# giolucasd/ssrl-vit-mae-jepa

Hardware: AMD Instinct MI355X
Metric: images/sec pretrain step (fwd+bwd+opt), ViT-S/8 96px MAE, 1/2/4/8 MI355X (higher is better)
Workload: dtype bf16; 1 GPU; ViT-S/8 96px MAE (enc 384x12x6h, dec 192x2x6h, mask_ratio 0.75), batch 2000/GPU, full step; global_batch=2000, per_gpu_batch=2000, parallelism=dp1

## Files before the change

### __graft_entry__.py

```python
from __future__ import annotations

import os
import subprocess
import sys
from pathlib import Path

ROOT = Path(__file__).resolve().parent
if str(ROOT) not in sys.path:
    sys.path.insert(0, str(ROOT))


def build() -> None:
    env = dict(os.environ)
    env.setdefault("HIPCC", "/opt/rocm/bin/hipcc")
    jobs = str(min(8, os.cpu_count() or 1))
    subprocess.run(["make", "-C", str(ROOT / "ssrl_vit_mae_jepa_amd" / "csrc"), "-j", jobs, "ARCH=gfx950"], check=True, env=env)
    subprocess.run(["bash", str(ROOT / "tools" / "build_dbg_lib.sh"), "vmcnt0"], check=True, env=dict(env, JOBS=jobs))
    import oracle.mae_oracle
    import ssrl_vit_mae_jepa_amd
    print("build ok:", ssrl_vit_mae_jepa_amd.LIB_PATH)


def smoke() -> None:
    import torch
    from oracle import mae_oracle as O
    from ssrl_vit_mae_jepa_amd import MaskedAutoencoder

    torch.set_float32_matmul_precision("highest")
    dev = torch.device("cuda:0")
    cfg = O.YAML_TINY
    B = 4
    params = O.init_params(cfg, 73)
    O.randomize_params(params)
    images = O.synthetic_images(B, cfg)
    noise = O.make_noise(B, cfg.sequence_length, torch.Generator().manual_seed(74))
    loss_ref, grads_ref, aux = O.loss_and_grads(params, cfg, images, noise)
    for precision, tol in (("fp32", 1e-4), ("bf16", 2e-2)):
        model = MaskedAutoencoder(
            dict(image_size=cfg.image_size, patch_size=cfg.patch_size, in_chans=cfg.in_chans, engine_precision=precision),
            dict(embed_dim=cfg.embed_dim, depth=cfg.depth, num_heads=cfg.num_heads),
            dict(decoder_embed_dim=cfg.decoder_embed_dim, decoder_depth=cfg.decoder_depth, decoder_num_heads=cfg.decoder_num_heads))
        model.load_state_dict(params)
        model = model.to(dev)
        loss, keep, mask = model.loss_and_grads(images.to(dev), noise.to(dev), return_indices=True)
        torch.cuda.synchronize()
        assert torch.equal(keep.cpu(), aux["idx_keep"]) and torch.equal(mask.cpu(), aux["idx_mask"]), "mask indices differ"
        rel = abs(loss.item() - loss_ref.item()) / abs(loss_ref.item())
        assert rel <= tol, f"{precision}: loss {loss.item()} vs oracle {loss_ref.item()} (rel {rel:.2e})"
        g = model.named_flat_views(model.flat_grads)
        gn = sum(float(v.double().pow(2).sum()) for v in g.values()) ** 0.5
        gr = sum(float(v.double().pow(2).sum()) for v in grads_ref.values()) ** 0.5
        assert abs(gn - gr) <= max(50 * tol, 1e-3) * gr, f"{precision}: grad norm {gn} vs {gr}"
        print(f"smoke {precision}: loss {loss.item():.6f} (oracle {loss_ref.item():.6f}, rel {rel:.1e}), |g| {gn:.5f} vs {gr:.5f}")


if __name__ == "__main__":
    build()
    if len(sys.argv) > 1 and sys.argv[1] == "smoke":
        smoke()
```

### ssrl_vit_mae_jepa_amd/csrc/k_attention_mfma.hip

```cpp
#include "gemm_mfma.h"

#ifndef MAE_ATT_DMA_POLICY
#define MAE_ATT_DMA_POLICY 0
#endif
#ifdef MAE_ATT_NT
#define AT_ST store4_nt
#else
#define AT_ST store4
#endif

namespace mae {

namespace {

constexpr float kLog2e = 1.4426950408889634f;

template <int HD>
struct AT {
  static constexpr int RS = HD * 2 + 32;
  static constexpr int NKS = HD / 32;
  static constexpr int NDT = HD / 16;
  static constexpr int CPR = HD / 8;
};

template <int HD>
__device__ __forceinline__ void stage_image(char* s, const bf16* g, int64_t gs, int T, int Tp) {
  for (int c = threadIdx.x; c < Tp * AT<HD>::CPR; c += blockDim.x) {
    const int row = c / AT<HD>::CPR, cc = c - row * AT<HD>::CPR;
    uint4 v = uint4{0, 0, 0, 0};
    if (row < T) v = *reinterpret_cast<const uint4*>(g + row * gs + cc * 8);
    *reinterpret_cast<uint4*>(s + row * AT<HD>::RS + cc * 16) = v;
  }
}

template <int HD>
__device__ __forceinline__ void stage_image_dma(char* s, int img_bytes, const bf16* g, int64_t gs, int T, int wave, int nwaves, int lane, int cprv) {
  constexpr int SPR = AT<HD>::RS / 16;
  for (int blk = wave; blk * 1024 < img_bytes; blk += nwaves) {
    const int slot = blk * 64 + lane;
    int row = slot / SPR, c = slot - row * SPR;
    row = row < T ? row : T - 1;
    c = c < cprv ? c : cprv - 1;
    __builtin_amdgcn_global_load_lds((const __attribute__((address_space(1))) void*)(g + row * gs + c * 8),
                                     (__attribute__((address_space(3))) void*)(s + blk * 1024), 16, 0, MAE_ATT_DMA_POLICY);
  }
}

template <int HD>
__device__ __forceinline__ void zero_pad_chunks(char* s, int rows, int cprv) {
  const int npad = AT<HD>::CPR - cprv;
  for (int i = threadIdx.x; i < rows * npad; i += blockDim.x) {
    const int row = i / npad, c = cprv + (i - row * npad);
    *reinterpret_cast<uint4*>(s + row * AT<HD>::RS + c * 16) = uint4{0, 0, 0, 0};
  }
}

template <int HD, bool CL>
__device__ __forceinline__ bf16x8 rowfrag(const char* s, int row0, int ks, int lane, int rmax) {
  const int row = CL ? min(row0 + (lane & 15), rmax) : row0 + (lane & 15);
  return *reinterpret_cast<const bf16x8*>(s + row * AT<HD>::RS + (ks * 32 + 8 * (lane >> 4)) * 2);
}

template <int HD, bool CL>
__device__ __forceinline__ bf16x8 trfrag(const char* s, int j0, int c0, int lane, int rmax) {
  const int g = lane >> 4, q = (lane & 15) >> 2, p = lane & 3;
  const int r = j0 + 4 * g + q;
  const char* a = s + (CL ? min(r, rmax) : r) * AT<HD>::RS + (c0 + 4 * p) * 2;
  const char* a2 = CL ? s + min(r + 16, rmax) * AT<HD>::RS + (c0 + 4 * p) * 2 : a + 16 * AT<HD>::RS;
  const bf16x4 lo = __builtin_amdgcn_ds_read_tr16_b64_v4bf16((__attribute__((address_space(3))) bf16x4*)(a));
  const bf16x4 hi = __builtin_amdgcn_ds_read_tr16_b64_v4bf16((__attribute__((address_space(3))) bf16x4*)(a2));
  return bf16x8{lo[0], lo[1], lo[2], lo[3], hi[0], hi[1], hi[2], hi[3]};
}

__device__ __forceinline__ bf16x8 pack8(const f32x4& a, const f32x4& b) {
  return bf16x8{(bf16)a[0], (bf16)a[1], (bf16)a[2], (bf16)a[3], (bf16)b[0], (bf16)b[1], (bf16)b[2], (bf16)b[3]};
}

__device__ __forceinline__ float group_max(float v) {
  auto a = __builtin_amdgcn_permlane16_swap(__float_as_uint(v), __float_as_uint(v), false, false);
  v = fmaxf(__uint_as_float(a[0]), __uint_as_float(a[1]));
  auto b = __builtin_amdgcn_permlane32_swap(__float_as_uint(v), __float_as_uint(v), false, false);
  return fmaxf(__uint_as_float(b[0]), __uint_as_float(b[1]));
}
__device__ __forceinline__ float group_sum(float v) {
  auto a = __builtin_amdgcn_permlane16_swap(__float_as_uint(v), __float_as_uint(v), false, false);
  v = __uint_as_float(a[0]) + __uint_as_float(a[1]);
  auto b = __builtin_amdgcn_permlane32_swap(__float_as_uint(v), __float_as_uint(v), false, false);
  return __uint_as_float(b[0]) + __uint_as_float(b[1]);
}

}

__device__ __forceinline__ void first_generation_stagger(int stagger, int gen1) {
  if (stagger > 0 && (int)blockIdx.x >= 256 && (int)blockIdx.x < gen1) {
    const uint64_t t0 = wall_clock64(), wait = (uint64_t)(blockIdx.x >> 8) * stagger;
    while (wall_clock64() - t0 < wait) __builtin_amdgcn_s_sleep(4);
  }
}

__device__ __forceinline__ int att_block(int remap) {
  if (!remap) return (int)blockIdx.x;
  const int nb = (int)gridDim.x, bid = (int)blockIdx.x;
  const int q = nb >> 3, r = nb & 7, xcd = bid & 7, loc = bid >> 3;
  return (xcd < r ? xcd * (q + 1) : r * (q + 1) + (xcd - r) * q) + loc;
}

template <int HD> struct FwdCap { static constexpr int v = 512; };
template <int NCH> struct BwdCap { static constexpr int v = NCH == 0 ? 1024 : 512; };

template <int HD>
__device__ __forceinline__ bf16x8 rowfrag_global(const bf16* g, int64_t gs, int row0, int ks, int lane, int T) {
  int row = row0 + (lane & 15);
  row = row < T ? row : T - 1;
  return *reinterpret_cast<const bf16x8*>(g + row * gs + ks * 32 + 8 * (lane >> 4));
}

template <int HD, int NCH, bool FQ = false>
__global__ void __launch_bounds__(FwdCap<HD>::v) attn_fwd_mfma_kernel(const bf16* __restrict__ qkv, int T, int Tp, int H, float scale,
                                                            bf16* __restrict__ out, float* __restrict__ lse, int stagger, int gen1, int hdv, int remap) {
  extern __shared__ __attribute__((aligned(16))) char smem[];
  first_generation_stagger(stagger, gen1);
  constexpr bool CL = NCH >= 1 && NCH <= 3;
  const int Ti = CL ? (T + 15) & ~15 : Tp, rmax = Ti - 1;
  const int img = (Ti * AT<HD>::RS + 1023) & ~1023;
  char* sQ = smem;
  char* sK = FQ ? smem : sQ + img;
  char* sV = sK + img;
  const int vb = att_block(remap);
  const int b = vb / H, h = vb - b * H;
  const int64_t gs = 3ll * H * hdv;
  const int cprv = hdv >> 3;
  const bf16* base = qkv + (int64_t)b * T * gs + h * hdv;
  const int lane = threadIdx.x & 63, nwaves = blockDim.x >> 6;
  const int wave = __builtin_amdgcn_readfirstlane(threadIdx.x >> 6);
  if (!FQ) stage_image_dma<HD>(sQ, img, base, gs, T, wave, nwaves, lane, cprv);
  stage_image_dma<HD>(sK, img, base + (int64_t)H * hdv, gs, T, wave, nwaves, lane, cprv);
  stage_image_dma<HD>(sV, img, base + 2ll * H * hdv, gs, T, wave, nwaves, lane, cprv);
  asm volatile("s_waitcnt vmcnt(0)" ::: "memory");
  if (hdv < HD) {
    if (!FQ) zero_pad_chunks<HD>(sQ, Ti, cprv);
    zero_pad_chunks<HD>(sK, Ti, cprv);
    zero_pad_chunks<HD>(sV, Ti, cprv);
  }
  __syncthreads();
  const int g = lane >> 4, i = lane & 15;
  const float sl2 = scale * kLog2e;
  const int nq = (T + 15) >> 4, nchunks = NCH > 0 ? NCH : (Tp >> 5);
  for (int qt = wave; qt < nq; qt += nwaves) {
    bf16x8 qf[AT<HD>::NKS];
#pragma unroll
    for (int ks = 0; ks < AT<HD>::NKS; ++ks) qf[ks] = FQ ? rowfrag_global<HD>(base, gs, qt * 16, ks, lane, T) : rowfrag<HD, CL>(sQ, qt * 16, ks, lane, rmax);
    f32x4 oacc[AT<HD>::NDT];
#pragma unroll
    for (int dt = 0; dt < AT<HD>::NDT; ++dt) oacc[dt] = f32x4{0.f, 0.f, 0.f, 0.f};
    float m = -INFINITY, lsum = 0.f;
    if constexpr (NCH > 0) {
      constexpr int NC = NCH > 0 ? NCH : 1;
      f32x4 s0[NC], s1[NC];
#pragma unroll
      for (int c = 0; c < NC; ++c) {
        s0[c] = f32x4{0.f, 0.f, 0.f, 0.f}; s1[c] = s0[c];
#pragma unroll
        for (int ks = 0; ks < AT<HD>::NKS; ++ks) {
          s0[c] = __builtin_amdgcn_mfma_f32_16x16x32_bf16(rowfrag<HD, CL>(sK, c * 32, ks, lane, rmax), qf[ks], s0[c], 0, 0, 0);
          s1[c] = __builtin_amdgcn_mfma_f32_16x16x32_bf16(rowfrag<HD, CL>(sK, c * 32 + 16, ks, lane, rmax), qf[ks], s1[c], 0, 0, 0);
        }
      }
      {
        const int j0 = (NC - 1) * 32 + 4 * g;
#pragma unroll
        for (int r = 0; r < 4; ++r) {
          if (j0 + r >= T) s0[NC - 1][r] = -INFINITY;
          if (j0 + 16 + r >= T) s1[NC - 1][r] = -INFINITY;
        }
      }
      float mc = -INFINITY;
#pragma unroll
      for (int c = 0; c < NC; ++c)
        mc = fmaxf(mc, fmaxf(fmaxf(fmaxf(s0[c][0], s0[c][1]), fmaxf(s0[c][2], s0[c][3])), fmaxf(fmaxf(s1[c][0], s1[c][1]), fmaxf(s1[c][2], s1[c][3]))));
      m = group_max(mc);
      const float mn2 = m * sl2;
#pragma unroll
      for (int c = 0; c < NC; ++c) {
#pragma unroll
        for (int r = 0; r < 4; ++r) {
          s0[c][r] = __builtin_amdgcn_exp2f(fmaf(s0[c][r], sl2, -mn2));
          s1[c][r] = __builtin_amdgcn_exp2f(fmaf(s1[c][r], sl2, -mn2));
          lsum += s0[c][r] + s1[c][r];
        }
        const bf16x8 pf = pack8(s0[c], s1[c]);
#pragma unroll
        for (int dt = 0; dt < AT<HD>::NDT; ++dt)
          oacc[dt] = __builtin_amdgcn_mfma_f32_16x16x32_bf16(trfrag<HD, CL>(sV, c * 32, dt * 16, lane, rmax), pf, oacc[dt], 0, 0, 0);
      }
    } else {
    for (int c = 0; c < nchunks; ++c) {
      f32x4 s0 = {0.f, 0.f, 0.f, 0.f}, s1 = {0.f, 0.f, 0.f, 0.f};
#pragma unroll
      for (int ks = 0; ks < AT<HD>::NKS; ++ks) {
        s0 = __builtin_amdgcn_mfma_f32_16x16x32_bf16(rowfrag<HD, CL>(sK, c * 32, ks, lane, rmax), qf[ks], s0, 0, 0, 0);
        s1 = __builtin_amdgcn_mfma_f32_16x16x32_bf16(rowfrag<HD, CL>(sK, c * 32 + 16, ks, lane, rmax), qf[ks], s1, 0, 0, 0);
      }
      const int j0 = c * 32 + 4 * g;
      if (c * 32 + 32 > T) {
#pragma unroll
        for (int r = 0; r < 4; ++r) {
          if (j0 + r >= T) s0[r] = -INFINITY;
          if (j0 + 16 + r >= T) s1[r] = -INFINITY;
        }
      }
      float mc = fmaxf(fmaxf(fmaxf(s0[0], s0[1]), fmaxf(s0[2], s0[3])), fmaxf(fmaxf(s1[0], s1[1]), fmaxf(s1[2], s1[3])));
      mc = group_max(mc);
      const float mn = fmaxf(m, mc);
      const float mn2 = mn * sl2;
      const float alpha = __builtin_amdgcn_exp2f(m * sl2 - mn2);
      float ps = 0.f;
#pragma unroll
      for (int r = 0; r < 4; ++r) {
        s0[r] = __builtin_amdgcn_exp2f(fmaf(s0[r], sl2, -mn2));
        s1[r] = __builtin_amdgcn_exp2f(fmaf(s1[r], sl2, -mn2));
        ps += s0[r] + s1[r];
      }
      lsum = lsum * alpha + ps;
      const bf16x8 pf = pack8(s0, s1);
#pragma unroll
      for (int dt = 0; dt < AT<HD>::NDT; ++dt) {
        oacc[dt] *= alpha;
        oacc[dt] = __builtin_amdgcn_mfma_f32_16x16x32_bf16(trfrag<HD, CL>(sV, c * 32, dt * 16, lane, rmax), pf, oacc[dt], 0, 0, 0);
      }
      m = mn;
    }
    }
    lsum = group_sum(lsum);
    const float inv = 1.0f / lsum;
    const int tq = qt * 16 + i;
    if (tq < T) {
      bf16* po = out + ((int64_t)b * T + tq) * H * hdv + h * hdv + 4 * g;
#pragma unroll
      for (int dt = 0; dt < AT<HD>::NDT; ++dt)
        if (dt * 16 + 4 * g < hdv) AT_ST(po + dt * 16, oacc[dt] * inv);
      if (g == 0) lse[((int64_t)b * H + h) * T + tq] = m * scale + __logf(lsum);
    }
  }
}

template <int HD, int NCH, int PH = 0>
__global__ void __launch_bounds__(BwdCap<NCH>::v) attn_bwd_mfma_kernel(const bf16* __restrict__ qkv, const bf16* __restrict__ out,
                                                            const bf16* __restrict__ d_out, const float* __restrict__ lse, int T,
                                                            int Tp, int H, float scale, bf16* __restrict__ d_qkv, int stagger, int gen1, int hdv, int remap) {
  extern __shared__ __attribute__((aligned(16))) char smem[];
  first_generation_stagger(stagger, gen1);
  constexpr bool CL = NCH >= 1 && NCH <= 3;
  const int Ti = CL ? (T + 15) & ~15 : Tp, rmax = Ti - 1;
  const int img = (Ti * AT<HD>::RS + 1023) & ~1023;
  char* sQ = smem;
  char* sK = PH == 1 ? smem : sQ + img;
  char* sV = sK + img;
  char* sdO = PH == 2 ? smem + img : sV + img;
  float* sLse = reinterpret_cast<float*>(smem + (PH == 0 ? 4 : 2) * img);
  float* sD = sLse + Tp;
  const int vb = att_block(remap);
  const int b = vb / H, h = vb - b * H;
  const int64_t gs = 3ll * H * hdv, os = (int64_t)H * hdv;
  const int cprv = hdv >> 3;
  const bf16* base = qkv + (int64_t)b * T * gs + h * hdv;
  const bf16* obase = out + (int64_t)b * T * os + h * hdv;
  const bf16* dobase = d_out + (int64_t)b * T * os + h * hdv;
  bf16* dbase = d_qkv + (int64_t)b * T * gs + h * hdv;
  const int lane = threadIdx.x & 63, nwaves = blockDim.x >> 6;
  const int wave = __builtin_amdgcn_readfirstlane(threadIdx.x >> 6);
  if (PH != 1) stage_image_dma<HD>(sQ, img, base, gs, T, wave, nwaves, lane, cprv);
  if (PH != 2) stage_image_dma<HD>(sK, img, base + os, gs, T, wave, nwaves, lane, cprv);
  if (PH != 2) stage_image_dma<HD>(sV, img, base + 2 * os, gs, T, wave, nwaves, lane, cprv);
  if (PH != 1) stage_image_dma<HD>(sdO, img, dobase, os, T, wave, nwaves, lane, cprv);
  constexpr bool DPM = NCH > 0 && PH == 0;
  constexpr int CPR = AT<HD>::CPR, PF = 4;
  const int total = Tp * CPR;
  const bool pf = !DPM && PH == 0 && total <= PF * (int)blockDim.x;
  if (DPM) {
    for (int t = threadIdx.x; t < Tp; t += blockDim.x) {
      sLse[t] = t < T ? lse[((int64_t)b * H + h) * T + t] * kLog2e : 1e30f;
      sD[t] = 0.f;
    }
  }
  bf16x8 o_pf[PF];
  float l_pf[PF];
  if (pf) {
#pragma unroll
    for (int it = 0; it < PF; ++it) {
      const int idx = it * blockDim.x + threadIdx.x;
      const int t = idx / CPR, cc = idx - t * CPR;
      const bool live = idx < total && t < T && cc < cprv;
      const int tc = live ? t : 0;
      o_pf[it] = *reinterpret_cast<const bf16x8*>(obase + tc * os + (live ? cc : 0) * 8);
      l_pf[it] = lse[((int64_t)b * H + h) * T + tc];
    }
  }
  asm volatile("s_waitcnt vmcnt(0)" ::: "memory");
  if (hdv < HD) {
    if (PH != 1) zero_pad_chunks<HD>(sQ, Ti, cprv);
    if (PH != 2) zero_pad_chunks<HD>(sK, Ti, cprv);
    if (PH != 2) zero_pad_chunks<HD>(sV, Ti, cprv);
    if (PH != 1) zero_pad_chunks<HD>(sdO, Ti, cprv);
  }
  __syncthreads();
  if (pf) {
#pragma unroll
    for (int it = 0; it < PF; ++it) {
      const int idx = it * blockDim.x + threadIdx.x;
      const int t = idx / CPR, cc = idx - t * CPR;
      float D = 0.f;
      if (idx < total && t < T && cc < cprv) {
        const bf16x8 a = *reinterpret_cast<const bf16x8*>(sdO + t * AT<HD>::RS + cc * 16);
#pragma unroll
        for (int e = 0; e < 8; ++e) D = fmaf((float)a[e], (float)o_pf[it][e], D);
      }
#pragma unroll
      for (int off = CPR / 2; off > 0; off >>= 1) D += __shfl_xor(D, off, 64);
      if (idx < total && cc == 0) {
        sD[t] = D;
        sLse[t] = t < T ? l_pf[it] * kLog2e : 1e30f;
      }
    }
  } else if (!DPM) {
    for (int base = 0; base < total; base += blockDim.x) {
      const int idx = base + threadIdx.x;
      const int t = idx / CPR, cc = idx - t * CPR;
      float D = 0.f;
      if (idx < total && t < T && cc < cprv) {
        const bf16x8 a = PH == 1 ? *reinterpret_cast<const bf16x8*>(dobase + t * os + cc * 8) : *reinterpret_cast<const bf16x8*>(sdO + t * AT<HD>::RS + cc * 16);
        const bf16x8 o = *reinterpret_cast<const bf16x8*>(obase + t * os + cc * 8);
#pragma unroll
        for (int e = 0; e < 8; ++e) D = fmaf((float)a[e], (float)o[e], D);
      }
#pragma unroll
      for (int off = CPR / 2; off > 0; off >>= 1) D += __shfl_xor(D, off, 64);
      if (idx < total && cc == 0) {
        sD[t] = D;
        sLse[t] = t < T ? lse[((int64_t)b * H + h) * T + t] * kLog2e : 1e30f;
      }
    }
  }
  if (!DPM) __syncthreads();
  const int g = lane >> 4, i = lane & 15;
  const float sl2 = scale * kLog2e;
  const int nt16 = (T + 15) >> 4, nchunks = NCH > 0 ? NCH : (Tp >> 5);

#ifdef MAE_DBG_ATT_NO_A
  if (T < 0)
#endif
  if (PH != 2)
  for (int qt = wave; qt < nt16; qt += nwaves) {
    bf16x8 qf[AT<HD>::NKS], dof[AT<HD>::NKS];
#pragma unroll
    for (int ks = 0; ks < AT<HD>::NKS; ++ks) {
      qf[ks] = PH == 1 ? rowfrag_global<HD>(base, gs, qt * 16, ks, lane, T) : rowfrag<HD, CL>(sQ, qt * 16, ks, lane, rmax);
      dof[ks] = PH == 1 ? rowfrag_global<HD>(dobase, os, qt * 16, ks, lane, T) : rowfrag<HD, CL>(sdO, qt * 16, ks, lane, rmax);
    }
    const float li = sLse[qt * 16 + i];
    f32x4 dq[AT<HD>::NDT];
#pragma unroll
    for (int dt = 0; dt < AT<HD>::NDT; ++dt) dq[dt] = f32x4{0.f, 0.f, 0.f, 0.f};
    if constexpr (DPM) {
      constexpr int NC = NCH > 0 ? NCH : 1;
      f32x4 P0[NC], P1[NC], G0[NC], G1[NC];
      float dpart = 0.f;
#pragma unroll
      for (int c = 0; c < NC; ++c) {
        f32x4 s0 = {0.f, 0.f, 0.f, 0.f}, s1 = s0;
        G0[c] = s0; G1[c] = s0;
#pragma unroll
        for (int ks = 0; ks < AT<HD>::NKS; ++ks) {
          s0 = __builtin_amdgcn_mfma_f32_16x16x32_bf16(rowfrag<HD, CL>(sK, c * 32, ks, lane, rmax), qf[ks], s0, 0, 0, 0);
          s1 = __builtin_amdgcn_mfma_f32_16x16x32_bf16(rowfrag<HD, CL>(sK, c * 32 + 16, ks, lane, rmax), qf[ks], s1, 0, 0, 0);
          G0[c] = __builtin_amdgcn_mfma_f32_16x16x32_bf16(rowfrag<HD, CL>(sV, c * 32, ks, lane, rmax), dof[ks], G0[c], 0, 0, 0);
          G1[c] = __builtin_amdgcn_mfma_f32_16x16x32_bf16(rowfrag<HD, CL>(sV, c * 32 + 16, ks, lane, rmax), dof[ks], G1[c], 0, 0, 0);
        }
        if (c == NC - 1) {
          const int j0 = c * 32 + 4 * g;
#pragma unroll
          for (int r = 0; r < 4; ++r) {
            if (j0 + r >= T) s0[r] = -INFINITY;
            if (j0 + 16 + r >= T) s1[r] = -INFINITY;
          }
        }
#pragma unroll
        for (int r = 0; r < 4; ++r) {
          P0[c][r] = __builtin_amdgcn_exp2f(fmaf(s0[r], sl2, -li));
          P1[c][r] = __builtin_amdgcn_exp2f(fmaf(s1[r], sl2, -li));
          dpart = fmaf(P0[c][r], G0[c][r], dpart);
          dpart = fmaf(P1[c][r], G1[c][r], dpart);
        }
      }
      const float Di = group_sum(dpart);
      if (g == 0) sD[qt * 16 + i] = Di;
#pragma unroll
      for (int c = 0; c < NC; ++c) {
        f32x4 d0, d1;
#pragma unroll
        for (int r = 0; r < 4; ++r) {
          d0[r] = P0[c][r] * (G0[c][r] - Di);
          d1[r] = P1[c][r] * (G1[c][r] - Di);
        }
        const bf16x8 dsf = pack8(d0, d1);
#pragma unroll
        for (int dt = 0; dt < AT<HD>::NDT; ++dt)
          dq[dt] = __builtin_amdgcn_mfma_f32_16x16x32_bf16(trfrag<HD, CL>(sK, c * 32, dt * 16, lane, rmax), dsf, dq[dt], 0, 0, 0);
      }
    } else {
    const float Di = sD[qt * 16 + i];
#pragma unroll
    for (int c = 0; c < nchunks; ++c) {
      f32x4 s0 = {0.f, 0.f, 0.f, 0.f}, s1 = s0, p0 = s0, p1 = s0;
#pragma unroll
      for (int ks = 0; ks < AT<HD>::NKS; ++ks) {
        s0 = __builtin_amdgcn_mfma_f32_16x16x32_bf16(rowfrag<HD, CL>(sK, c * 32, ks, lane, rmax), qf[ks], s0, 0, 0, 0);
        s1 = __builtin_amdgcn_mfma_f32_16x16x32_bf16(rowfrag<HD, CL>(sK, c * 32 + 16, ks, lane, rmax), qf[ks], s1, 0, 0, 0);
        p0 = __builtin_amdgcn_mfma_f32_16x16x32_bf16(rowfrag<HD, CL>(sV, c * 32, ks, lane, rmax), dof[ks], p0, 0, 0, 0);
        p1 = __builtin_amdgcn_mfma_f32_16x16x32_bf16(rowfrag<HD, CL>(sV, c * 32 + 16, ks, lane, rmax), dof[ks], p1, 0, 0, 0);
      }
      const int j0 = c * 32 + 4 * g;
      if (NCH > 0 ? c == NCH - 1 : c * 32 + 32 > T) {
#pragma unroll
        for (int r = 0; r < 4; ++r) {
          if (j0 + r >= T) s0[r] = -INFINITY;
          if (j0 + 16 + r >= T) s1[r] = -INFINITY;
        }
      }
#pragma unroll
      for (int r = 0; r < 4; ++r) {
        const float pa = __builtin_amdgcn_exp2f(fmaf(s0[r], sl2, -li));
        const float pb = __builtin_amdgcn_exp2f(fmaf(s1[r], sl2, -li));
        s0[r] = pa * (p0[r] - Di);
        s1[r] = pb * (p1[r] - Di);
      }
      const bf16x8 dsf = pack8(s0, s1);
#pragma unroll
      for (int dt = 0; dt < AT<HD>::NDT; ++dt)
        dq[dt] = __builtin_amdgcn_mfma_f32_16x16x32_bf16(trfrag<HD, CL>(sK, c * 32, dt * 16, lane, rmax), dsf, dq[dt], 0, 0, 0);
    }
    }
    const int tq = qt * 16 + i;
    if (tq < T) {
#pragma unroll
      for (int dt = 0; dt < AT<HD>::NDT; ++dt)
        if (dt * 16 + 4 * g < hdv) AT_ST(dbase + tq * gs + dt * 16 + 4 * g, dq[dt] * scale);
    }
  }
  if (DPM) __syncthreads();

#ifdef MAE_DBG_ATT_NO_B
  if (T < 0)
#endif
  if (PH != 1)
  for (int jt = wave; jt < nt16; jt += nwaves) {
    bf16x8 kf[AT<HD>::NKS], vf[AT<HD>::NKS];
#pragma unroll
    for (int ks = 0; ks < AT<HD>::NKS; ++ks) {
      kf[ks] = PH == 2 ? rowfrag_global<HD>(base + os, gs, jt * 16, ks, lane, T) : rowfrag<HD, CL>(sK, jt * 16, ks, lane, rmax);
      vf[ks] = PH == 2 ? rowfrag_global<HD>(base + 2 * os, gs, jt * 16, ks, lane, T) : rowfrag<HD, CL>(sV, jt * 16, ks, lane, rmax);
    }
    f32x4 dk[AT<HD>::NDT], dv[AT<HD>::NDT];
#pragma unroll
    for (int dt = 0; dt < AT<HD>::NDT; ++dt) { dk[dt] = f32x4{0.f, 0.f, 0.f, 0.f}; dv[dt] = dk[dt]; }
#pragma unroll
    for (int c = 0; c < nchunks; ++c) {
      f32x4 s0 = {0.f, 0.f, 0.f, 0.f}, s1 = s0, p0 = s0, p1 = s0;
#pragma unroll
      for (int ks = 0; ks < AT<HD>::NKS; ++ks) {
        s0 = __builtin_amdgcn_mfma_f32_16x16x32_bf16(rowfrag<HD, CL>(sQ, c * 32, ks, lane, rmax), kf[ks], s0, 0, 0, 0);
        s1 = __builtin_amdgcn_mfma_f32_16x16x32_bf16(rowfrag<HD, CL>(sQ, c * 32 + 16, ks, lane, rmax), kf[ks], s1, 0, 0, 0);
        p0 = __builtin_amdgcn_mfma_f32_16x16x32_bf16(rowfrag<HD, CL>(sdO, c * 32, ks, lane, rmax), vf[ks], p0, 0, 0, 0);
        p1 = __builtin_amdgcn_mfma_f32_16x16x32_bf16(rowfrag<HD, CL>(sdO, c * 32 + 16, ks, lane, rmax), vf[ks], p1, 0, 0, 0);
      }
      const f32x4 l0 = load4(sLse + c * 32 + 4 * g), l1 = load4(sLse + c * 32 + 16 + 4 * g);
      const f32x4 D0 = load4(sD + c * 32 + 4 * g), D1 = load4(sD + c * 32 + 16 + 4 * g);
      f32x4 ds0, ds1;
#pragma unroll
      for (int r = 0; r < 4; ++r) {
        s0[r] = __builtin_amdgcn_exp2f(fmaf(s0[r], sl2, -l0[r]));
        s1[r] = __builtin_amdgcn_exp2f(fmaf(s1[r], sl2, -l1[r]));
        ds0[r] = s0[r] * (p0[r] - D0[r]);
        ds1[r] = s1[r] * (p1[r] - D1[r]);
      }
      const bf16x8 pf = pack8(s0, s1), dsf = pack8(ds0, ds1);
#pragma unroll
      for (int dt = 0; dt < AT<HD>::NDT; ++dt) {
        dv[dt] = __builtin_amdgcn_mfma_f32_16x16x32_bf16(trfrag<HD, CL>(sdO, c * 32, dt * 16, lane, rmax), pf, dv[dt], 0, 0, 0);
        dk[dt] = __builtin_amdgcn_mfma_f32_16x16x32_bf16(trfrag<HD, CL>(sQ, c * 32, dt * 16, lane, rmax), dsf, dk[dt], 0, 0, 0);
      }
    }
    const int tj = jt * 16 + i;
    if (tj < T) {
#pragma unroll
      for (int dt = 0; dt < AT<HD>::NDT; ++dt) {
        if (dt * 16 + 4 * g < hdv) {
          AT_ST(dbase + tj * gs + os + dt * 16 + 4 * g, dk[dt] * scale);
          AT_ST(dbase + tj * gs + 2 * os + dt * 16 + 4 * g, dv[dt]);
        }
      }
    }
  }
}

static int attn_waves(int T, int max_threads) {
  const int nt = (T + 15) / 16, maxw = max_threads / 64;
  const int passes = (nt + maxw - 1) / maxw;
  return (nt + passes - 1) / passes;
}

static int attn_remap() {
  static const int v = [] { const char* e = getenv("MAE_ATT_XCD"); return e ? atoi(e) : 1; }();
  return v;
}
static int attn_stagger() {
  static const int v = [] { const char* e = getenv("MAE_ATT_STAGGER"); return e ? atoi(e) : 0; }();
  return v;
}
static int attn_resident(size_t lds, int threads) {
  const int by_lds = (int)((160 * 1024) / lds), by_waves = 32 / (threads / 64);
  return std::max(1, std::min(std::min(by_lds, by_waves), 8));
}

static bool attn_supported(int T, int H, int hd) {
  return (hd == 24 || hd == 32 || hd == 64) && T >= 1 && T <= 1024 && ((int64_t)H * hd) % 8 == 0;
}

template <int HD, int NCH>
static int launch_attn_fwd(const bf16* qkv, int B, int T, int Tp, int H, int hdv, size_t lds, float scale, bf16* out, float* lse, hipStream_t s) {
  auto kern = attn_fwd_mfma_kernel<HD, NCH>;
  MAE_HIP(hipFuncSetAttribute((const void*)kern, hipFuncAttributeMaxDynamicSharedMemorySize, (int)lds));
  hipLaunchKernelGGL(kern, dim3((unsigned)B * H), dim3(64 * attn_waves(T, FwdCap<HD>::v)), lds, s, qkv, T, Tp, H, scale, out, lse, attn_stagger(), 256 * attn_resident(lds, 64 * attn_waves(T, FwdCap<HD>::v)), hdv, attn_remap());
  MAE_LAUNCH_CHECK();
  return 0;
}
template <int HD, int NCH>
static int launch_attn_bwd(const bf16* qkv, const bf16* out, const bf16* d_out, const float* lse, int B, int T, int Tp, int H, int hdv, size_t lds,
                           float scale, bf16* d_qkv, hipStream_t s) {
  auto kern = attn_bwd_mfma_kernel<HD, NCH>;
  static const int lds_pad = [] { const char* e = getenv("MAE_ATT_LDS_PAD"); return e ? atoi(e) : 0; }();
  lds += (size_t)lds_pad;
  MAE_HIP(hipFuncSetAttribute((const void*)kern, hipFuncAttributeMaxDynamicSharedMemorySize, (int)lds));
  hipLaunchKernelGGL(kern, dim3((unsigned)B * H), dim3(64 * attn_waves(T, BwdCap<NCH>::v)), lds, s, qkv, out, d_out, lse, T, Tp, H, scale, d_qkv, attn_stagger(), 256 * attn_resident(lds, 64 * attn_waves(T, BwdCap<NCH>::v)), hdv, attn_remap());
  MAE_LAUNCH_CHECK();
  return 0;
}
template <int HD>
static int launch_attn_bwd_split(const bf16* qkv, const bf16* out, const bf16* d_out, const float* lse, int B, int T, int Tp, int H, int hdv, size_t lds,
                                 float scale, bf16* d_qkv, hipStream_t s) {
  const int threads = 64 * attn_waves(T, BwdCap<0>::v);
  auto k1 = attn_bwd_mfma_kernel<HD, 0, 1>;
  auto k2 = attn_bwd_mfma_kernel<HD, 0, 2>;
  MAE_HIP(hipFuncSetAttribute((const void*)k1, hipFuncAttributeMaxDynamicSharedMemorySize, (int)lds));
  MAE_HIP(hipFuncSetAttribute((const void*)k2, hipFuncAttributeMaxDynamicSharedMemorySize, (int)lds));
  hipLaunchKernelGGL(k1, dim3((unsigned)B * H), dim3(threads), lds, s, qkv, out, d_out, lse, T, Tp, H, scale, d_qkv, 0, 0, hdv, attn_remap());
  MAE_LAUNCH_CHECK();
  hipLaunchKernelGGL(k2, dim3((unsigned)B * H), dim3(threads), lds, s, qkv, out, d_out, lse, T, Tp, H, scale, d_qkv, 0, 0, hdv, attn_remap());
  MAE_LAUNCH_CHECK();
  return 0;
}
#define ATTN_DISPATCH(FN, BIG, ...)                                         \
  switch (hdt * 100 + (Tp >> 5)) {                                          \
    case 6401: return FN<64, 1>(__VA_ARGS__);                               \
    case 6402: return FN<64, 2>(__VA_ARGS__);                               \
    case 6403: return FN<64, 3>(__VA_ARGS__);                               \
    case 6405: return FN<64, BIG>(__VA_ARGS__);   \
    case 3201: return FN<32, 1>(__VA_ARGS__);                               \
    case 3202: return FN<32, 2>(__VA_ARGS__);                               \
    case 3203: return FN<32, 3>(__VA_ARGS__);                               \
    case 3205: return FN<32, BIG>(__VA_ARGS__);                             \
    default: return hdt == 64 ? FN<64, 0>(__VA_ARGS__) : FN<32, 0>(__VA_ARGS__); \
  }

template <int HD>
static int launch_attn_fwd_fq(const bf16* qkv, int B, int T, int Tp, int H, int hdv, size_t lds, float scale, bf16* out, float* lse, hipStream_t s) {
  auto kern = attn_fwd_mfma_kernel<HD, 0, true>;
  MAE_HIP(hipFuncSetAttribute((const void*)kern, hipFuncAttributeMaxDynamicSharedMemorySize, (int)lds));
  hipLaunchKernelGGL(kern, dim3((unsigned)B * H), dim3(64 * attn_waves(T, FwdCap<HD>::v)), lds, s, qkv, T, Tp, H, scale, out, lse, 0, 0, hdv, attn_remap());
  MAE_LAUNCH_CHECK();
  return 0;
}

int mfma_attention_fwd(const bf16* qkv, int B, int T, int H, int hd, bf16* out, float* lse, hipStream_t s) {
  if (!attn_supported(T, H, hd) || (((uintptr_t)qkv | (uintptr_t)out) & 15)) return MFMA_UNSUPPORTED;
  const int Tp = (int)round_up(T, 32), hdt = hd == 24 ? 32 : hd;
  const size_t img = (size_t)round_up(((Tp >> 5) <= 3 ? round_up((int64_t)T, 16) : (int64_t)Tp) * (hdt * 2 + 32), 1024);
  const size_t lds = 3 * img;
  const float scale = 1.0f / sqrtf((float)hd);
  if (lds > 160 * 1024) {
    if (2 * img > 160 * 1024 || hd != hdt) return MFMA_UNSUPPORTED;
    return hdt == 64 ? launch_attn_fwd_fq<64>(qkv, B, T, Tp, H, hd, 2 * img, scale, out, lse, s) : launch_attn_fwd_fq<32>(qkv, B, T, Tp, H, hd, 2 * img, scale, out, lse, s);
  }
  ATTN_DISPATCH(launch_attn_fwd, 5, qkv, B, T, Tp, H, hd, lds, scale, out, lse, s)
}

int mfma_attention_bwd(const bf16* qkv, const bf16* out, const bf16* d_out, const float* lse, int B, int T, int H, int hd,
                       bf16* d_qkv, hipStream_t s) {
  if (!attn_supported(T, H, hd) || (((uintptr_t)qkv | (uintptr_t)out | (uintptr_t)d_out | (uintptr_t)d_qkv) & 15)) return MFMA_UNSUPPORTED;
  const int Tp = (int)round_up(T, 32), hdt = hd == 24 ? 32 : hd;
  const size_t img = (size_t)round_up(((Tp >> 5) <= 3 ? round_up((int64_t)T, 16) : (int64_t)Tp) * (hdt * 2 + 32), 1024);
  const size_t lds = 4 * img + (size_t)2 * Tp * 4;
  const float scale = 1.0f / sqrtf((float)hd);
  if (lds > 160 * 1024) {
    const size_t lds2 = 2 * img + (size_t)2 * Tp * 4;
    if (lds2 > 160 * 1024 || hd != hdt) return MFMA_UNSUPPORTED;
    return hdt == 64 ? launch_attn_bwd_split<64>(qkv, out, d_out, lse, B, T, Tp, H, hd, lds2, scale, d_qkv, s)
                     : launch_attn_bwd_split<32>(qkv, out, d_out, lse, B, T, Tp, H, hd, lds2, scale, d_qkv, s);
  }
  ATTN_DISPATCH(launch_attn_bwd, 0, qkv, out, d_out, lse, B, T, Tp, H, hd, lds, scale, d_qkv, s)
}

}
```

Baseline: 91550 images/s.

## Replace padded LDS rows in attention kernels with XOR-swizzled layout per config

Attention Q/K/V/dO images in LDS switch from rows padded by 32 bytes to unpadded rows with an XOR swizzle on the 16-byte chunk index. Padding is kept only for selected (head dim, chunk count) configurations. The aim is to avoid bank conflicts while shrinking the LDS footprint so more blocks can be resident. Staging, fragment reads, transposed reads and LDS sizing are all updated to match. The residency estimate for the stagger path now accounts for register usage, and a debug build variant that forces padding is added.

```diff
diff --git a/__graft_entry__.py b/__graft_entry__.py
--- a/__graft_entry__.py
+++ b/__graft_entry__.py
@@ -16,6 +16,7 @@
     jobs = str(min(8, os.cpu_count() or 1))
     subprocess.run(["make", "-C", str(ROOT / "ssrl_vit_mae_jepa_amd" / "csrc"), "-j", jobs, "ARCH=gfx950"], check=True, env=env)
     subprocess.run(["bash", str(ROOT / "tools" / "build_dbg_lib.sh"), "vmcnt0"], check=True, env=dict(env, JOBS=jobs))
+    subprocess.run(["bash", str(ROOT / "tools" / "build_dbg_lib.sh"), "att_padded"], check=True, env=dict(env, JOBS=jobs))
     import oracle.mae_oracle
     import ssrl_vit_mae_jepa_amd
     print("build ok:", ssrl_vit_mae_jepa_amd.LIB_PATH)
diff --git a/ssrl_vit_mae_jepa_amd/csrc/k_attention_mfma.hip b/ssrl_vit_mae_jepa_amd/csrc/k_attention_mfma.hip
--- a/ssrl_vit_mae_jepa_amd/csrc/k_attention_mfma.hip
+++ b/ssrl_vit_mae_jepa_amd/csrc/k_attention_mfma.hip
@@ -15,30 +15,38 @@
 
 constexpr float kLog2e = 1.4426950408889634f;
 
-template <int HD>
+template <int HD, bool PAD>
 struct AT {
-  static constexpr int RS = HD * 2 + 32;
+  static constexpr int RS = HD * 2 + (PAD ? 32 : 0);
   static constexpr int NKS = HD / 32;
   static constexpr int NDT = HD / 16;
   static constexpr int CPR = HD / 8;
+  static constexpr int SPR = RS / 16;
+  static __device__ __forceinline__ int sw(int row) { return PAD ? 0 : HD == 64 ? (row & 6) << 4 : (row & 4) << 3; }
 };
-
-template <int HD>
+#ifdef MAE_DBG_ATT_PADDED
+template <int HD, int NCH> struct FwdPad { static constexpr bool v = true; };
+template <int HD, int NCH> struct BwdPad { static constexpr bool v = true; };
+#else
+template <int HD, int NCH> struct FwdPad { static constexpr bool v = HD == 64 && NCH == 5; };
+template <int HD, int NCH> struct BwdPad { static constexpr bool v = (HD == 64 && NCH == 2) || (HD == 32 && NCH == 3); };
+#endif
+
+template <class L>
 __device__ __forceinline__ void stage_image(char* s, const bf16* g, int64_t gs, int T, int Tp) {
-  for (int c = threadIdx.x; c < Tp * AT<HD>::CPR; c += blockDim.x) {
-    const int row = c / AT<HD>::CPR, cc = c - row * AT<HD>::CPR;
+  for (int c = threadIdx.x; c < Tp * L::CPR; c += blockDim.x) {
+    const int row = c / L::CPR, cc = c - row * L::CPR;
     uint4 v = uint4{0, 0, 0, 0};
     if (row < T) v = *reinterpret_cast<const uint4*>(g + row * gs + cc * 8);
-    *reinterpret_cast<uint4*>(s + row * AT<HD>::RS + cc * 16) = v;
-  }
-}
-
-template <int HD>
+    *reinterpret_cast<uint4*>(s + row * L::RS + ((cc * 16) ^ L::sw(row))) = v;
+  }
+}
+
+template <class L>
 __device__ __forceinline__ void stage_image_dma(char* s, int img_bytes, const bf16* g, int64_t gs, int T, int wave, int nwaves, int lane, int cprv) {
-  constexpr int SPR = AT<HD>::RS / 16;
   for (int blk = wave; blk * 1024 < img_bytes; blk += nwaves) {
     const int slot = blk * 64 + lane;
-    int row = slot / SPR, c = slot - row * SPR;
+    int row = slot / L::SPR, c = (slot - row * L::SPR) ^ (L::sw(row) >> 4);
     row = row < T ? row : T - 1;
     c = c < cprv ? c : cprv - 1;
     __builtin_amdgcn_global_load_lds((const __attribute__((address_space(1))) void*)(g + row * gs + c * 8),
@@ -46,27 +54,30 @@
   }
 }
 
-template <int HD>
+template <class L>
 __device__ __forceinline__ void zero_pad_chunks(char* s, int rows, int cprv) {
-  const int npad = AT<HD>::CPR - cprv;
+  const int npad = L::CPR - cprv;
   for (int i = threadIdx.x; i < rows * npad; i += blockDim.x) {
     const int row = i / npad, c = cprv + (i - row * npad);
-    *reinterpret_cast<uint4*>(s + row * AT<HD>::RS + c * 16) = uint4{0, 0, 0, 0};
-  }
-}
-
-template <int HD, bool CL>
+    *reinterpret_cast<uint4*>(s + row * L::RS + ((c * 16) ^ L::sw(row))) = uint4{0, 0, 0, 0};
+  }
+}
+
+template <class L, int CLR>
 __device__ __forceinline__ bf16x8 rowfrag(const char* s, int row0, int ks, int lane, int rmax) {
-  const int row = CL ? min(row0 + (lane & 15), rmax) : row0 + (lane & 15);
-  return *reinterpret_cast<const bf16x8*>(s + row * AT<HD>::RS + (ks * 32 + 8 * (lane >> 4)) * 2);
-}
-
-template <int HD, bool CL>
+  const bool cl = CLR > 0 && row0 >= CLR;
+  const int row = cl ? min(row0 + (lane & 15), rmax) : row0 + (lane & 15);
+  return *reinterpret_cast<const bf16x8*>(s + row * L::RS + (((ks * 32 + 8 * (lane >> 4)) * 2) ^ L::sw(cl ? row : lane & 15)));
+}
+
+template <class L, int CLR>
 __device__ __forceinline__ bf16x8 trfrag(const char* s, int j0, int c0, int lane, int rmax) {
   const int g = lane >> 4, q = (lane & 15) >> 2, p = lane & 3;
   const int r = j0 + 4 * g + q;
-  const char* a = s + (CL ? min(r, rmax) : r) * AT<HD>::RS + (c0 + 4 * p) * 2;
-  const char* a2 = CL ? s + min(r + 16, rmax) * AT<HD>::RS + (c0 + 4 * p) * 2 : a + 16 * AT<HD>::RS;
+  const bool cl = CLR > 0 && j0 + 16 >= CLR;
+  const int r2 = cl ? min(r + 16, rmax) : r + 16;
+  const char* a = s + r * L::RS + (((c0 + 4 * p) * 2) ^ L::sw(4 * g + q));
+  const char* a2 = cl ? s + r2 * L::RS + (((c0 + 4 * p) * 2) ^ L::sw(r2)) : a + 16 * L::RS;
   const bf16x4 lo = __builtin_amdgcn_ds_read_tr16_b64_v4bf16((__attribute__((address_space(3))) bf16x4*)(a));
   const bf16x4 hi = __builtin_amdgcn_ds_read_tr16_b64_v4bf16((__attribute__((address_space(3))) bf16x4*)(a2));
   return bf16x8{lo[0], lo[1], lo[2], lo[3], hi[0], hi[1], hi[2], hi[3]};
@@ -106,7 +117,10 @@
 }
 
 template <int HD> struct FwdCap { static constexpr int v = 512; };
-template <int NCH> struct BwdCap { static constexpr int v = NCH == 0 ? 1024 : 512; };
+#ifndef MAE_ATT_BWD32_LOOP_THREADS
+#define MAE_ATT_BWD32_LOOP_THREADS 512
+#endif
+template <int HD, int NCH, int PH = 0> struct BwdCap { static constexpr int v = NCH != 0 ? 512 : (HD == 32 && PH == 0) ? MAE_ATT_BWD32_LOOP_THREADS : 1024; };
 
 template <int HD>
 __device__ __forceinline__ bf16x8 rowfrag_global(const bf16* g, int64_t gs, int row0, int ks, int lane, int T) {
@@ -121,8 +135,10 @@
   extern __shared__ __attribute__((aligned(16))) char smem[];
   first_generation_stagger(stagger, gen1);
   constexpr bool CL = NCH >= 1 && NCH <= 3;
+  constexpr int CLR = CL ? NCH * 32 - 16 : 0;
+  using L = AT<HD, FwdPad<HD, NCH>::v>;
   const int Ti = CL ? (T + 15) & ~15 : Tp, rmax = Ti - 1;
-  const int img = (Ti * AT<HD>::RS + 1023) & ~1023;
+  const int img = (Ti * L::RS + 1023) & ~1023;
   char* sQ = smem;
   char* sK = FQ ? smem : sQ + img;
   char* sV = sK + img;
@@ -133,26 +149,26 @@
   const bf16* base = qkv + (int64_t)b * T * gs + h * hdv;
   const int lane = threadIdx.x & 63, nwaves = blockDim.x >> 6;
   const int wave = __builtin_amdgcn_readfirstlane(threadIdx.x >> 6);
-  if (!FQ) stage_image_dma<HD>(sQ, img, base, gs, T, wave, nwaves, lane, cprv);
-  stage_image_dma<HD>(sK, img, base + (int64_t)H * hdv, gs, T, wave, nwaves, lane, cprv);
-  stage_image_dma<HD>(sV, img, base + 2ll * H * hdv, gs, T, wave, nwaves, lane, cprv);
+  if (!FQ) stage_image_dma<L>(sQ, img, base, gs, T, wave, nwaves, lane, cprv);
+  stage_image_dma<L>(sK, img, base + (int64_t)H * hdv, gs, T, wave, nwaves, lane, cprv);
+  stage_image_dma<L>(sV, img, base + 2ll * H * hdv, gs, T, wave, nwaves, lane, cprv);
   asm volatile("s_waitcnt vmcnt(0)" ::: "memory");
   if (hdv < HD) {
-    if (!FQ) zero_pad_chunks<HD>(sQ, Ti, cprv);
-    zero_pad_chunks<HD>(sK, Ti, cprv);
-    zero_pad_chunks<HD>(sV, Ti, cprv);
+    if (!FQ) zero_pad_chunks<L>(sQ, Ti, cprv);
+    zero_pad_chunks<L>(sK, Ti, cprv);
+    zero_pad_chunks<L>(sV, Ti, cprv);
   }
   __syncthreads();
   const int g = lane >> 4, i = lane & 15;
   const float sl2 = scale * kLog2e;
   const int nq = (T + 15) >> 4, nchunks = NCH > 0 ? NCH : (Tp >> 5);
   for (int qt = wave; qt < nq; qt += nwaves) {
-    bf16x8 qf[AT<HD>::NKS];
-#pragma unroll
-    for (int ks = 0; ks < AT<HD>::NKS; ++ks) qf[ks] = FQ ? rowfrag_global<HD>(base, gs, qt * 16, ks, lane, T) : rowfrag<HD, CL>(sQ, qt * 16, ks, lane, rmax);
-    f32x4 oacc[AT<HD>::NDT];
-#pragma unroll
-    for (int dt = 0; dt < AT<HD>::NDT; ++dt) oacc[dt] = f32x4{0.f, 0.f, 0.f, 0.f};
+    bf16x8 qf[L::NKS];
+#pragma unroll
+    for (int ks = 0; ks < L::NKS; ++ks) qf[ks] = FQ ? rowfrag_global<HD>(base, gs, qt * 16, ks, lane, T) : rowfrag<L, CLR>(sQ, qt * 16, ks, lane, rmax);
+    f32x4 oacc[L::NDT];
+#pragma unroll
+    for (int dt = 0; dt < L::NDT; ++dt) oacc[dt] = f32x4{0.f, 0.f, 0.f, 0.f};
     float m = -INFINITY, lsum = 0.f;
     if constexpr (NCH > 0) {
       constexpr int NC = NCH > 0 ? NCH : 1;
@@ -161,9 +177,9 @@
       for (int c = 0; c < NC; ++c) {
         s0[c] = f32x4{0.f, 0.f, 0.f, 0.f}; s1[c] = s0[c];
 #pragma unroll
-        for (int ks = 0; ks < AT<HD>::NKS; ++ks) {
-          s0[c] = __builtin_amdgcn_mfma_f32_16x16x32_bf16(rowfrag<HD, CL>(sK, c * 32, ks, lane, rmax), qf[ks], s0[c], 0, 0, 0);
-          s1[c] = __builtin_amdgcn_mfma_f32_16x16x32_bf16(rowfrag<HD, CL>(sK, c * 32 + 16, ks, lane, rmax), qf[ks], s1[c], 0, 0, 0);
+        for (int ks = 0; ks < L::NKS; ++ks) {
+          s0[c] = __builtin_amdgcn_mfma_f32_16x16x32_bf16(rowfrag<L, CLR>(sK, c * 32, ks, lane, rmax), qf[ks], s0[c], 0, 0, 0);
+          s1[c] = __builtin_amdgcn_mfma_f32_16x16x32_bf16(rowfrag<L, CLR>(sK, c * 32 + 16, ks, lane, rmax), qf[ks], s1[c], 0, 0, 0);
         }
       }
       {
@@ -190,16 +206,16 @@
         }
         const bf16x8 pf = pack8(s0[c], s1[c]);
 #pragma unroll
-        for (int dt = 0; dt < AT<HD>::NDT; ++dt)
-          oacc[dt] = __builtin_amdgcn_mfma_f32_16x16x32_bf16(trfrag<HD, CL>(sV, c * 32, dt * 16, lane, rmax), pf, oacc[dt], 0, 0, 0);
+        for (int dt = 0; dt < L::NDT; ++dt)
+          oacc[dt] = __builtin_amdgcn_mfma_f32_16x16x32_bf16(trfrag<L, CLR>(sV, c * 32, dt * 16, lane, rmax), pf, oacc[dt], 0, 0, 0);
       }
     } else {
     for (int c = 0; c < nchunks; ++c) {
       f32x4 s0 = {0.f, 0.f, 0.f, 0.f}, s1 = {0.f, 0.f, 0.f, 0.f};
 #pragma unroll
-      for (int ks = 0; ks < AT<HD>::NKS; ++ks) {
-        s0 = __builtin_amdgcn_mfma_f32_16x16x32_bf16(rowfrag<HD, CL>(sK, c * 32, ks, lane, rmax), qf[ks], s0, 0, 0, 0);
-        s1 = __builtin_amdgcn_mfma_f32_16x16x32_bf16(rowfrag<HD, CL>(sK, c * 32 + 16, ks, lane, rmax), qf[ks], s1, 0, 0, 0);
+      for (int ks = 0; ks < L::NKS; ++ks) {
+        s0 = __builtin_amdgcn_mfma_f32_16x16x32_bf16(rowfrag<L, CLR>(sK, c * 32, ks, lane, rmax), qf[ks], s0, 0, 0, 0);
+        s1 = __builtin_amdgcn_mfma_f32_16x16x32_bf16(rowfrag<L, CLR>(sK, c * 32 + 16, ks, lane, rmax), qf[ks], s1, 0, 0, 0);
       }
       const int j0 = c * 32 + 4 * g;
       if (c * 32 + 32 > T) {
@@ -224,9 +240,9 @@
       lsum = lsum * alpha + ps;
       const bf16x8 pf = pack8(s0, s1);
 #pragma unroll
-      for (int dt = 0; dt < AT<HD>::NDT; ++dt) {
+      for (int dt = 0; dt < L::NDT; ++dt) {
         oacc[dt] *= alpha;
-        oacc[dt] = __builtin_amdgcn_mfma_f32_16x16x32_bf16(trfrag<HD, CL>(sV, c * 32, dt * 16, lane, rmax), pf, oacc[dt], 0, 0, 0);
+        oacc[dt] = __builtin_amdgcn_mfma_f32_16x16x32_bf16(trfrag<L, CLR>(sV, c * 32, dt * 16, lane, rmax), pf, oacc[dt], 0, 0, 0);
       }
       m = mn;
     }
@@ -237,7 +253,7 @@
     if (tq < T) {
       bf16* po = out + ((int64_t)b * T + tq) * H * hdv + h * hdv + 4 * g;
 #pragma unroll
-      for (int dt = 0; dt < AT<HD>::NDT; ++dt)
+      for (int dt = 0; dt < L::NDT; ++dt)
         if (dt * 16 + 4 * g < hdv) AT_ST(po + dt * 16, oacc[dt] * inv);
       if (g == 0) lse[((int64_t)b * H + h) * T + tq] = m * scale + __logf(lsum);
     }
@@ -245,14 +261,16 @@
 }
 
 template <int HD, int NCH, int PH = 0>
-__global__ void __launch_bounds__(BwdCap<NCH>::v) attn_bwd_mfma_kernel(const bf16* __restrict__ qkv, const bf16* __restrict__ out,
+__global__ void __launch_bounds__((BwdCap<HD, NCH, PH>::v)) attn_bwd_mfma_kernel(const bf16* __restrict__ qkv, const bf16* __restrict__ out,
                                                             const bf16* __restrict__ d_out, const float* __restrict__ lse, int T,
                                                             int Tp, int H, float scale, bf16* __restrict__ d_qkv, int stagger, int gen1, int hdv, int remap) {
   extern __shared__ __attribute__((aligned(16))) char smem[];
   first_generation_stagger(stagger, gen1);
   constexpr bool CL = NCH >= 1 && NCH <= 3;
+  constexpr int CLR = CL ? NCH * 32 - 16 : 0;
+  using L = AT<HD, BwdPad<HD, NCH>::v>;
   const int Ti = CL ? (T + 15) & ~15 : Tp, rmax = Ti - 1;
-  const int img = (Ti * AT<HD>::RS + 1023) & ~1023;
+  const int img = (Ti * L::RS + 1023) & ~1023;
   char* sQ = smem;
   char* sK = PH == 1 ? smem : sQ + img;
   char* sV = sK + img;
@@ -269,12 +287,12 @@
   bf16* dbase = d_qkv + (int64_t)b * T * gs + h * hdv;
   const int lane = threadIdx.x & 63, nwaves = blockDim.x >> 6;
   const int wave = __builtin_amdgcn_readfirstlane(threadIdx.x >> 6);
-  if (PH != 1) stage_image_dma<HD>(sQ, img, base, gs, T, wave, nwaves, lane, cprv);
-  if (PH != 2) stage_image_dma<HD>(sK, img, base + os, gs, T, wave, nwaves, lane, cprv);
-  if (PH != 2) stage_image_dma<HD>(sV, img, base + 2 * os, gs, T, wave, nwaves, lane, cprv);
-  if (PH != 1) stage_image_dma<HD>(sdO, img, dobase, os, T, wave, nwaves, lane, cprv);
+  if (PH != 1) stage_image_dma<L>(sQ, img, base, gs, T, wave, nwaves, lane, cprv);
+  if (PH != 2) stage_image_dma<L>(sK, img, base + os, gs, T, wave, nwaves, lane, cprv);
+  if (PH != 2) stage_image_dma<L>(sV, img, base + 2 * os, gs, T, wave, nwaves, lane, cprv);
+  if (PH != 1) stage_image_dma<L>(sdO, img, dobase, os, T, wave, nwaves, lane, cprv);
   constexpr bool DPM = NCH > 0 && PH == 0;
-  constexpr int CPR = AT<HD>::CPR, PF = 4;
+  constexpr int CPR = L::CPR, PF = 4;
   const int total = Tp * CPR;
   const bool pf = !DPM && PH == 0 && total <= PF * (int)blockDim.x;
   if (DPM) {
@@ -298,10 +316,10 @@
   }
   asm volatile("s_waitcnt vmcnt(0)" ::: "memory");
   if (hdv < HD) {
-    if (PH != 1) zero_pad_chunks<HD>(sQ, Ti, cprv);
-    if (PH != 2) zero_pad_chunks<HD>(sK, Ti, cprv);
-    if (PH != 2) zero_pad_chunks<HD>(sV, Ti, cprv);
-    if (PH != 1) zero_pad_chunks<HD>(sdO, Ti, cprv);
+    if (PH != 1) zero_pad_chunks<L>(sQ, Ti, cprv);
+    if (PH != 2) zero_pad_chunks<L>(sK, Ti, cprv);
+    if (PH != 2) zero_pad_chunks<L>(sV, Ti, cprv);
+    if (PH != 1) zero_pad_chunks<L>(sdO, Ti, cprv);
   }
   __syncthreads();
   if (pf) {
@@ -311,7 +329,7 @@
       const int t = idx / CPR, cc = idx - t * CPR;
       float D = 0.f;
       if (idx < total && t < T && cc < cprv) {
-        const bf16x8 a = *reinterpret_cast<const bf16x8*>(sdO + t * AT<HD>::RS + cc * 16);
+        const bf16x8 a = *reinterpret_cast<const bf16x8*>(sdO + t * L::RS + ((cc * 16) ^ L::sw(t)));
 #pragma unroll
         for (int e = 0; e < 8; ++e) D = fmaf((float)a[e], (float)o_pf[it][e], D);
       }
@@ -328,7 +346,7 @@
       const int t = idx / CPR, cc = idx - t * CPR;
       float D = 0.f;
       if (idx < total && t < T && cc < cprv) {
-        const bf16x8 a = PH == 1 ? *reinterpret_cast<const bf16x8*>(dobase + t * os + cc * 8) : *reinterpret_cast<const bf16x8*>(sdO + t * AT<HD>::RS + cc * 16);
+        const bf16x8 a = PH == 1 ? *reinterpret_cast<const bf16x8*>(dobase + t * os + cc * 8) : *reinterpret_cast<const bf16x8*>(sdO + t * L::RS + ((cc * 16) ^ L::sw(t)));
         const bf16x8 o = *reinterpret_cast<const bf16x8*>(obase + t * os + cc * 8);
 #pragma unroll
         for (int e = 0; e < 8; ++e) D = fmaf((float)a[e], (float)o[e], D);
@@ -351,16 +369,16 @@
 #endif
   if (PH != 2)
   for (int qt = wave; qt < nt16; qt += nwaves) {
-    bf16x8 qf[AT<HD>::NKS], dof[AT<HD>::NKS];
-#pragma unroll
-    for (int ks = 0; ks < AT<HD>::NKS; ++ks) {
-      qf[ks] = PH == 1 ? rowfrag_global<HD>(base, gs, qt * 16, ks, lane, T) : rowfrag<HD, CL>(sQ, qt * 16, ks, lane, rmax);
-      dof[ks] = PH == 1 ? rowfrag_global<HD>(dobase, os, qt * 16, ks, lane, T) : rowfrag<HD, CL>(sdO, qt * 16, ks, lane, rmax);
+    bf16x8 qf[L::NKS], dof[L::NKS];
+#pragma unroll
+    for (int ks = 0; ks < L::NKS; ++ks) {
+      qf[ks] = PH == 1 ? rowfrag_global<HD>(base, gs, qt * 16, ks, lane, T) : rowfrag<L, CLR>(sQ, qt * 16, ks, lane, rmax);
+      dof[ks] = PH == 1 ? rowfrag_global<HD>(dobase, os, qt * 16, ks, lane, T) : rowfrag<L, CLR>(sdO, qt * 16, ks, lane, rmax);
     }
     const float li = sLse[qt * 16 + i];
-    f32x4 dq[AT<HD>::NDT];
-#pragma unroll
-    for (int dt = 0; dt < AT<HD>::NDT; ++dt) dq[dt] = f32x4{0.f, 0.f, 0.f, 0.f};
+    f32x4 dq[L::NDT];
+#pragma unroll
+    for (int dt = 0; dt < L::NDT; ++dt) dq[dt] = f32x4{0.f, 0.f, 0.f, 0.f};
     if constexpr (DPM) {
       constexpr int NC = NCH > 0 ? NCH : 1;
       f32x4 P0[NC], P1[NC], G0[NC], G1[NC];
@@ -370,11 +388,11 @@
         f32x4 s0 = {0.f, 0.f, 0.f, 0.f}, s1 = s0;
         G0[c] = s0; G1[c] = s0;
 #pragma unroll
-        for (int ks = 0; ks < AT<HD>::NKS; ++ks) {
-          s0 = __builtin_amdgcn_mfma_f32_16x16x32_bf16(rowfrag<HD, CL>(sK, c * 32, ks, lane, rmax), qf[ks], s0, 0, 0, 0);
-          s1 = __builtin_amdgcn_mfma_f32_16x16x32_bf16(rowfrag<HD, CL>(sK, c * 32 + 16, ks, lane, rmax), qf[ks], s1, 0, 0, 0);
-          G0[c] = __builtin_amdgcn_mfma_f32_16x16x32_bf16(rowfrag<HD, CL>(sV, c * 32, ks, lane, rmax), dof[ks], G0[c], 0, 0, 0);
-          G1[c] = __builtin_amdgcn_mfma_f32_16x16x32_bf16(rowfrag<HD, CL>(sV, c * 32 + 16, ks, lane, rmax), dof[ks], G1[c], 0, 0, 0);
+        for (int ks = 0; ks < L::NKS; ++ks) {
+          s0 = __builtin_amdgcn_mfma_f32_16x16x32_bf16(rowfrag<L, CLR>(sK, c * 32, ks, lane, rmax), qf[ks], s0, 0, 0, 0);
+          s1 = __builtin_amdgcn_mfma_f32_16x16x32_bf16(rowfrag<L, CLR>(sK, c * 32 + 16, ks, lane, rmax), qf[ks], s1, 0, 0, 0);
+          G0[c] = __builtin_amdgcn_mfma_f32_16x16x32_bf16(rowfrag<L, CLR>(sV, c * 32, ks, lane, rmax), dof[ks], G0[c], 0, 0, 0);
+          G1[c] = __builtin_amdgcn_mfma_f32_16x16x32_bf16(rowfrag<L, CLR>(sV, c * 32 + 16, ks, lane, rmax), dof[ks], G1[c], 0, 0, 0);
         }
         if (c == NC - 1) {
           const int j0 = c * 32 + 4 * g;
@@ -404,8 +422,8 @@
         }
         const bf16x8 dsf = pack8(d0, d1);
 #pragma unroll
-        for (int dt = 0; dt < AT<HD>::NDT; ++dt)
-          dq[dt] = __builtin_amdgcn_mfma_f32_16x16x32_bf16(trfrag<HD, CL>(sK, c * 32, dt * 16, lane, rmax), dsf, dq[dt], 0, 0, 0);
+        for (int dt = 0; dt < L::NDT; ++dt)
+          dq[dt] = __builtin_amdgcn_mfma_f32_16x16x32_bf16(trfrag<L, CLR>(sK, c * 32, dt * 16, lane, rmax), dsf, dq[dt], 0, 0, 0);
       }
     } else {
     const float Di = sD[qt * 16 + i];
@@ -413,11 +431,11 @@
     for (int c = 0; c < nchunks; ++c) {
       f32x4 s0 = {0.f, 0.f, 0.f, 0.f}, s1 = s0, p0 = s0, p1 = s0;
 #pragma unroll
-      for (int ks = 0; ks < AT<HD>::NKS; ++ks) {
-        s0 = __builtin_amdgcn_mfma_f32_16x16x32_bf16(rowfrag<HD, CL>(sK, c * 32, ks, lane, rmax), qf[ks], s0, 0, 0, 0);
-        s1 = __builtin_amdgcn_mfma_f32_16x16x32_bf16(rowfrag<HD, CL>(sK, c * 32 + 16, ks, lane, rmax), qf[ks], s1, 0, 0, 0);
-        p0 = __builtin_amdgcn_mfma_f32_16x16x32_bf16(rowfrag<HD, CL>(sV, c * 32, ks, lane, rmax), dof[ks], p0, 0, 0, 0);
-        p1 = __builtin_amdgcn_mfma_f32_16x16x32_bf16(rowfrag<HD, CL>(sV, c * 32 + 16, ks, lane, rmax), dof[ks], p1, 0, 0, 0);
+      for (int ks = 0; ks < L::NKS; ++ks) {
+        s0 = __builtin_amdgcn_mfma_f32_16x16x32_bf16(rowfrag<L, CLR>(sK, c * 32, ks, lane, rmax), qf[ks], s0, 0, 0, 0);
+        s1 = __builtin_amdgcn_mfma_f32_16x16x32_bf16(rowfrag<L, CLR>(sK, c * 32 + 16, ks, lane, rmax), qf[ks], s1, 0, 0, 0);
+        p0 = __builtin_amdgcn_mfma_f32_16x16x32_bf16(rowfrag<L, CLR>(sV, c * 32, ks, lane, rmax), dof[ks], p0, 0, 0, 0);
+        p1 = __builtin_amdgcn_mfma_f32_16x16x32_bf16(rowfrag<L, CLR>(sV, c * 32 + 16, ks, lane, rmax), dof[ks], p1, 0, 0, 0);
       }
       const int j0 = c * 32 + 4 * g;
       if (NCH > 0 ? c == NCH - 1 : c * 32 + 32 > T) {
@@ -436,14 +454,14 @@
       }
       const bf16x8 dsf = pack8(s0, s1);
 #pragma unroll
-      for (int dt = 0; dt < AT<HD>::NDT; ++dt)
-        dq[dt] = __builtin_amdgcn_mfma_f32_16x16x32_bf16(trfrag<HD, CL>(sK, c * 32, dt * 16, lane, rmax), dsf, dq[dt], 0, 0, 0);
+      for (int dt = 0; dt < L::NDT; ++dt)
+        dq[dt] = __builtin_amdgcn_mfma_f32_16x16x32_bf16(trfrag<L, CLR>(sK, c * 32, dt * 16, lane, rmax), dsf, dq[dt], 0, 0, 0);
     }
     }
     const int tq = qt * 16 + i;
     if (tq < T) {
 #pragma unroll
-      for (int dt = 0; dt < AT<HD>::NDT; ++dt)
+      for (int dt = 0; dt < L::NDT; ++dt)
         if (dt * 16 + 4 * g < hdv) AT_ST(dbase + tq * gs + dt * 16 + 4 * g, dq[dt] * scale);
     }
   }
@@ -454,24 +472,24 @@
 #endif
   if (PH != 1)
   for (int jt = wave; jt < nt16; jt += nwaves) {
-    bf16x8 kf[AT<HD>::NKS], vf[AT<HD>::NKS];
-#pragma unroll
-    for (int ks = 0; ks < AT<HD>::NKS; ++ks) {
-      kf[ks] = PH == 2 ? rowfrag_global<HD>(base + os, gs, jt * 16, ks, lane, T) : rowfrag<HD, CL>(sK, jt * 16, ks, lane, rmax);
-      vf[ks] = PH == 2 ? rowfrag_global<HD>(base + 2 * os, gs, jt * 16, ks, lane, T) : rowfrag<HD, CL>(sV, jt * 16, ks, lane, rmax);
-    }
-    f32x4 dk[AT<HD>::NDT], dv[AT<HD>::NDT];
-#pragma unroll
-    for (int dt = 0; dt < AT<HD>::NDT; ++dt) { dk[dt] = f32x4{0.f, 0.f, 0.f, 0.f}; dv[dt] = dk[dt]; }
+    bf16x8 kf[L::NKS], vf[L::NKS];
+#pragma unroll
+    for (int ks = 0; ks < L::NKS; ++ks) {
+      kf[ks] = PH == 2 ? rowfrag_global<HD>(base + os, gs, jt * 16, ks, lane, T) : rowfrag<L, CLR>(sK, jt * 16, ks, lane, rmax);
+      vf[ks] = PH == 2 ? rowfrag_global<HD>(base + 2 * os, gs, jt * 16, ks, lane, T) : rowfrag<L, CLR>(sV, jt * 16, ks, lane, rmax);
+    }
+    f32x4 dk[L::NDT], dv[L::NDT];
+#pragma unroll
+    for (int dt = 0; dt < L::NDT; ++dt) { dk[dt] = f32x4{0.f, 0.f, 0.f, 0.f}; dv[dt] = dk[dt]; }
 #pragma unroll
     for (int c = 0; c < nchunks; ++c) {
       f32x4 s0 = {0.f, 0.f, 0.f, 0.f}, s1 = s0, p0 = s0, p1 = s0;
 #pragma unroll
-      for (int ks = 0; ks < AT<HD>::NKS; ++ks) {
-        s0 = __builtin_amdgcn_mfma_f32_16x16x32_bf16(rowfrag<HD, CL>(sQ, c * 32, ks, lane, rmax), kf[ks], s0, 0, 0, 0);
-        s1 = __builtin_amdgcn_mfma_f32_16x16x32_bf16(rowfrag<HD, CL>(sQ, c * 32 + 16, ks, lane, rmax), kf[ks], s1, 0, 0, 0);
-        p0 = __builtin_amdgcn_mfma_f32_16x16x32_bf16(rowfrag<HD, CL>(sdO, c * 32, ks, lane, rmax), vf[ks], p0, 0, 0, 0);
-        p1 = __builtin_amdgcn_mfma_f32_16x16x32_bf16(rowfrag<HD, CL>(sdO, c * 32 + 16, ks, lane, rmax), vf[ks], p1, 0, 0, 0);
+      for (int ks = 0; ks < L::NKS; ++ks) {
+        s0 = __builtin_amdgcn_mfma_f32_16x16x32_bf16(rowfrag<L, CLR>(sQ, c * 32, ks, lane, rmax), kf[ks], s0, 0, 0, 0);
+        s1 = __builtin_amdgcn_mfma_f32_16x16x32_bf16(rowfrag<L, CLR>(sQ, c * 32 + 16, ks, lane, rmax), kf[ks], s1, 0, 0, 0);
+        p0 = __builtin_amdgcn_mfma_f32_16x16x32_bf16(rowfrag<L, CLR>(sdO, c * 32, ks, lane, rmax), vf[ks], p0, 0, 0, 0);
+        p1 = __builtin_amdgcn_mfma_f32_16x16x32_bf16(rowfrag<L, CLR>(sdO, c * 32 + 16, ks, lane, rmax), vf[ks], p1, 0, 0, 0);
       }
       const f32x4 l0 = load4(sLse + c * 32 + 4 * g), l1 = load4(sLse + c * 32 + 16 + 4 * g);
       const f32x4 D0 = load4(sD + c * 32 + 4 * g), D1 = load4(sD + c * 32 + 16 + 4 * g);
@@ -485,15 +503,15 @@
       }
       const bf16x8 pf = pack8(s0, s1), dsf = pack8(ds0, ds1);
 #pragma unroll
-      for (int dt = 0; dt < AT<HD>::NDT; ++dt) {
-        dv[dt] = __builtin_amdgcn_mfma_f32_16x16x32_bf16(trfrag<HD, CL>(sdO, c * 32, dt * 16, lane, rmax), pf, dv[dt], 0, 0, 0);
-        dk[dt] = __builtin_amdgcn_mfma_f32_16x16x32_bf16(trfrag<HD, CL>(sQ, c * 32, dt * 16, lane, rmax), dsf, dk[dt], 0, 0, 0);
+      for (int dt = 0; dt < L::NDT; ++dt) {
+        dv[dt] = __builtin_amdgcn_mfma_f32_16x16x32_bf16(trfrag<L, CLR>(sdO, c * 32, dt * 16, lane, rmax), pf, dv[dt], 0, 0, 0);
+        dk[dt] = __builtin_amdgcn_mfma_f32_16x16x32_bf16(trfrag<L, CLR>(sQ, c * 32, dt * 16, lane, rmax), dsf, dk[dt], 0, 0, 0);
       }
     }
     const int tj = jt * 16 + i;
     if (tj < T) {
 #pragma unroll
-      for (int dt = 0; dt < AT<HD>::NDT; ++dt) {
+      for (int dt = 0; dt < L::NDT; ++dt) {
         if (dt * 16 + 4 * g < hdv) {
           AT_ST(dbase + tj * gs + os + dt * 16 + 4 * g, dk[dt] * scale);
           AT_ST(dbase + tj * gs + 2 * os + dt * 16 + 4 * g, dv[dt]);
@@ -517,8 +535,11 @@
   static const int v = [] { const char* e = getenv("MAE_ATT_STAGGER"); return e ? atoi(e) : 0; }();
   return v;
 }
-static int attn_resident(size_t lds, int threads) {
-  const int by_lds = (int)((160 * 1024) / lds), by_waves = 32 / (threads / 64);
+static int attn_resident(const void* kern, size_t lds, int threads) {
+  hipFuncAttributes fa;
+  if (hipFuncGetAttributes(&fa, kern) != hipSuccess) { (void)hipGetLastError(); fa.numRegs = 128; }
+  const int alloc = std::max(8, (fa.numRegs + 7) & ~7), per_simd = std::min(8, 512 / alloc), waves = threads / 64;
+  const int by_lds = (int)((160 * 1024) / lds), by_waves = std::min(32, 4 * per_simd) / waves;
   return std::max(1, std::min(std::min(by_lds, by_waves), 8));
 }
 
@@ -526,29 +547,39 @@
   return (hd == 24 || hd == 32 || hd == 64) && T >= 1 && T <= 1024 && ((int64_t)H * hd) % 8 == 0;
 }
 
+static size_t attn_img_bytes(int T, int Tp, int rs) {
+  return (size_t)round_up(((Tp >> 5) <= 3 ? round_up((int64_t)T, 16) : (int64_t)Tp) * rs, 1024);
+}
+constexpr size_t kAttnLdsMax = 160 * 1024;
+
 template <int HD, int NCH>
-static int launch_attn_fwd(const bf16* qkv, int B, int T, int Tp, int H, int hdv, size_t lds, float scale, bf16* out, float* lse, hipStream_t s) {
+static int launch_attn_fwd(const bf16* qkv, int B, int T, int Tp, int H, int hdv, float scale, bf16* out, float* lse, hipStream_t s) {
   auto kern = attn_fwd_mfma_kernel<HD, NCH>;
+  const size_t lds = 3 * attn_img_bytes(T, Tp, AT<HD, FwdPad<HD, NCH>::v>::RS);
+  const int threads = 64 * attn_waves(T, FwdCap<HD>::v);
   MAE_HIP(hipFuncSetAttribute((const void*)kern, hipFuncAttributeMaxDynamicSharedMemorySize, (int)lds));
-  hipLaunchKernelGGL(kern, dim3((unsigned)B * H), dim3(64 * attn_waves(T, FwdCap<HD>::v)), lds, s, qkv, T, Tp, H, scale, out, lse, attn_stagger(), 256 * attn_resident(lds, 64 * attn_waves(T, FwdCap<HD>::v)), hdv, attn_remap());
+  hipLaunchKernelGGL(kern, dim3((unsigned)B * H), dim3(threads), lds, s, qkv, T, Tp, H, scale, out, lse, attn_stagger(),
+                     attn_stagger() > 0 ? 256 * attn_resident((const void*)kern, lds, threads) : 0, hdv, attn_remap());
   MAE_LAUNCH_CHECK();
   return 0;
 }
 template <int HD, int NCH>
-static int launch_attn_bwd(const bf16* qkv, const bf16* out, const bf16* d_out, const float* lse, int B, int T, int Tp, int H, int hdv, size_t lds,
+static int launch_attn_bwd(const bf16* qkv, const bf16* out, const bf16* d_out, const float* lse, int B, int T, int Tp, int H, int hdv,
                            float scale, bf16* d_qkv, hipStream_t s) {
   auto kern = attn_bwd_mfma_kernel<HD, NCH>;
   static const int lds_pad = [] { const char* e = getenv("MAE_ATT_LDS_PAD"); return e ? atoi(e) : 0; }();
-  lds += (size_t)lds_pad;
+  const size_t lds = 4 * attn_img_bytes(T, Tp, AT<HD, BwdPad<HD, NCH>::v>::RS) + (size_t)2 * Tp * 4 + (size_t)lds_pad;
+  const int threads = 64 * attn_waves(T, BwdCap<HD, NCH>::v);
   MAE_HIP(hipFuncSetAttribute((const void*)kern, hipFuncAttributeMaxDynamicSharedMemorySize, (int)lds));
-  hipLaunchKernelGGL(kern, dim3((unsigned)B * H), dim3(64 * attn_waves(T, BwdCap<NCH>::v)), lds, s, qkv, out, d_out, lse, T, Tp, H, scale, d_qkv, attn_stagger(), 256 * attn_resident(lds, 64 * attn_waves(T, BwdCap<NCH>::v)), hdv, attn_remap());
+  hipLaunchKernelGGL(kern, dim3((unsigned)B * H), dim3(threads), lds, s, qkv, out, d_out, lse, T, Tp, H, scale, d_qkv, attn_stagger(),
+                     attn_stagger() > 0 ? 256 * attn_resident((const void*)kern, lds, threads) : 0, hdv, attn_remap());
   MAE_LAUNCH_CHECK();
   return 0;
 }
 template <int HD>
 static int launch_attn_bwd_split(const bf16* qkv, const bf16* out, const bf16* d_out, const float* lse, int B, int T, int Tp, int H, int hdv, size_t lds,
                                  float scale, bf16* d_qkv, hipStream_t s) {
-  const int threads = 64 * attn_waves(T, BwdCap<0>::v);
+  const int threads = 64 * attn_waves(T, BwdCap<HD, 0, 1>::v);
   auto k1 = attn_bwd_mfma_kernel<HD, 0, 1>;
   auto k2 = attn_bwd_mfma_kernel<HD, 0, 2>;
   MAE_HIP(hipFuncSetAttribute((const void*)k1, hipFuncAttributeMaxDynamicSharedMemorySize, (int)lds));
@@ -584,30 +615,28 @@
 int mfma_attention_fwd(const bf16* qkv, int B, int T, int H, int hd, bf16* out, float* lse, hipStream_t s) {
   if (!attn_supported(T, H, hd) || (((uintptr_t)qkv | (uintptr_t)out) & 15)) return MFMA_UNSUPPORTED;
   const int Tp = (int)round_up(T, 32), hdt = hd == 24 ? 32 : hd;
-  const size_t img = (size_t)round_up(((Tp >> 5) <= 3 ? round_up((int64_t)T, 16) : (int64_t)Tp) * (hdt * 2 + 32), 1024);
-  const size_t lds = 3 * img;
+  const size_t img = attn_img_bytes(T, Tp, hdt == 64 ? AT<64, FwdPad<64, 0>::v>::RS : AT<32, FwdPad<32, 0>::v>::RS);
   const float scale = 1.0f / sqrtf((float)hd);
-  if (lds > 160 * 1024) {
-    if (2 * img > 160 * 1024 || hd != hdt) return MFMA_UNSUPPORTED;
+  if (3 * img > kAttnLdsMax) {
+    if (2 * img > kAttnLdsMax || hd != hdt) return MFMA_UNSUPPORTED;
     return hdt == 64 ? launch_attn_fwd_fq<64>(qkv, B, T, Tp, H, hd, 2 * img, scale, out, lse, s) : launch_attn_fwd_fq<32>(qkv, B, T, Tp, H, hd, 2 * img, scale, out, lse, s);
   }
-  ATTN_DISPATCH(launch_attn_fwd, 5, qkv, B, T, Tp, H, hd, lds, scale, out, lse, s)
+  ATTN_DISPATCH(launch_attn_fwd, 5, qkv, B, T, Tp, H, hd, scale, out, lse, s)
 }
 
 int mfma_attention_bwd(const bf16* qkv, const bf16* out, const bf16* d_out, const float* lse, int B, int T, int H, int hd,
                        bf16* d_qkv, hipStream_t s) {
   if (!attn_supported(T, H, hd) || (((uintptr_t)qkv | (uintptr_t)out | (uintptr_t)d_out | (uintptr_t)d_qkv) & 15)) return MFMA_UNSUPPORTED;
   const int Tp = (int)round_up(T, 32), hdt = hd == 24 ? 32 : hd;
-  const size_t img = (size_t)round_up(((Tp >> 5) <= 3 ? round_up((int64_t)T, 16) : (int64_t)Tp) * (hdt * 2 + 32), 1024);
-  const size_t lds = 4 * img + (size_t)2 * Tp * 4;
+  const size_t img = attn_img_bytes(T, Tp, hdt == 64 ? AT<64, BwdPad<64, 0>::v>::RS : AT<32, BwdPad<32, 0>::v>::RS);
   const float scale = 1.0f / sqrtf((float)hd);
-  if (lds > 160 * 1024) {
+  if (4 * img + (size_t)2 * Tp * 4 > kAttnLdsMax) {
     const size_t lds2 = 2 * img + (size_t)2 * Tp * 4;
-    if (lds2 > 160 * 1024 || hd != hdt) return MFMA_UNSUPPORTED;
+    if (lds2 > kAttnLdsMax || hd != hdt) return MFMA_UNSUPPORTED;
     return hdt == 64 ? launch_attn_bwd_split<64>(qkv, out, d_out, lse, B, T, Tp, H, hd, lds2, scale, d_qkv, s)
                      : launch_attn_bwd_split<32>(qkv, out, d_out, lse, B, T, Tp, H, hd, lds2, scale, d_qkv, s);
   }
-  ATTN_DISPATCH(launch_attn_bwd, 0, qkv, out, d_out, lse, B, T, Tp, H, hd, lds, scale, d_qkv, s)
-}
-
-}
+  ATTN_DISPATCH(launch_attn_bwd, 0, qkv, out, d_out, lse, B, T, Tp, H, hd, scale, d_qkv, s)
+}
+
+}
```

After: 92250 images/s (median of 6 runs). About the same (+0.8%).
